# cwkd/BiGCN

Measured on AMD Instinct MI355X. Metric: propagation-trees/sec fwd+bwd, batch=128, 5000-dim feats @ 1/2/4/8 MI355X, higher is better.
Workload: dtype f32

## Files before the change

### bigcn_amd/csrc/bgcn_csc_body.h

```cpp
#pragma once

#include "bgcn_internal.h"
#include "bgcn_sparse.h"

namespace bgcn {

__device__ __forceinline__ int spill_row_of(const int* pre, int nrows, int e) {
  int lo = 0, hi = nrows - 1;
  while (lo < hi) {
    const int mid = (lo + hi + 1) >> 1;
    if (pre[mid] <= e) lo = mid; else hi = mid - 1;
  }
  return lo;
}
template <class Fn>
__device__ __forceinline__ void for_spill(const SparseState& S, const int* pre, const int* off, int nrows,
                                          Fn f) {
  const int total = pre[nrows];
  for (int e0 = int(threadIdx.x); e0 < total; e0 += 4 * int(blockDim.x)) {
    int r[4];
    uint2 v[4];
#pragma unroll
    for (int u = 0; u < 4; ++u) {
      const int e = min(e0 + u * int(blockDim.x), total - 1);
      r[u] = spill_row_of(pre, nrows, e);
      v[u] = S.ovf[off[r[u]] + (e - pre[r[u]])];
    }
#pragma unroll
    for (int u = 0; u < 4; ++u)
      if (e0 + u * int(blockDim.x) < total) f(r[u], v[u]);
  }
}

__device__ inline void csc_hist_body(const SparseState& S, int bid, int32_t* hsm) {
  if (!use_sparse(S)) return;
  for (int64_t c = threadIdx.x; c < S.F; c += kRowBlock) hsm[c] = 0;
  const int64_t i = int64_t(bid) * kRowBlock + threadIdx.x;
  const int64_t ic = min<int64_t>(i, S.N - 1);
  const int nall = i < S.N ? S.nnz[ic] : 0;
  const int n = min(nall, kCap);
  int32_t cl[kCap];
#pragma unroll
  for (int q = 0; q < kCap / 4; ++q) {
    const int4 v = *reinterpret_cast<const int4*>(S.cols + ic * kCap + 4 * q);
    cl[4 * q] = v.x; cl[4 * q + 1] = v.y; cl[4 * q + 2] = v.z; cl[4 * q + 3] = v.w;
  }
  __syncthreads();
#pragma unroll
  for (int s = 0; s < kCap; ++s)
    if (s < n) atomicAdd(&hsm[cl[s]], 1);
  const int nsp = nall > kCap ? nall - kCap : 0;
  if (__syncthreads_or(nsp)) {
    __shared__ int pre[kRowBlock + 1], off[kRowBlock], wsum[kRowBlock / 64];
    const int lane = threadIdx.x & 63, wv = threadIdx.x >> 6;
    int x = nsp;
#pragma unroll
    for (int o = 1; o < 64; o <<= 1) {
      const int y = __shfl_up(x, o, 64);
      if (lane >= o) x += y;
    }
    if (lane == 63) wsum[wv] = x;
    __syncthreads();
    int base = 0, total = 0;
#pragma unroll
    for (int w = 0; w < kRowBlock / 64; ++w) {
      base += w < wv ? wsum[w] : 0;
      total += wsum[w];
    }
    pre[threadIdx.x] = base + x - nsp;
    off[threadIdx.x] = nsp ? S.ovf_off[ic] : 0;
    if (threadIdx.x == 0) pre[kRowBlock] = total;
    __syncthreads();
    for_spill(S, pre, off, kRowBlock, [&](int, uint2 v) { atomicAdd(&hsm[v.x], 1); });
  }
  __syncthreads();
  int32_t* out = S.hist + int64_t(bid) * S.F;
  for (int64_t c = threadIdx.x; c < S.F; c += kRowBlock) out[c] = hsm[c];
}

constexpr int kPrefixCols = 16, kPrefixSegs = 256 / kPrefixCols;
__device__ inline void csc_prefix_body(const SparseState& S, int R, int bid) {
  if (!use_sparse(S)) return;
  __shared__ int32_t part[kPrefixSegs][kPrefixCols];
  const int cl = threadIdx.x % kPrefixCols, q = threadIdx.x / kPrefixCols;
  const int64_t c = min<int64_t>(int64_t(bid) * kPrefixCols + cl, S.F - 1);
  const bool live = int64_t(bid) * kPrefixCols + cl < S.F;
  const int rq = (R + kPrefixSegs - 1) / kPrefixSegs, rb = q * rq, re = min(R, rb + rq);
  int32_t sum = 0;
  for (int r0 = rb; r0 < re; r0 += 8) {
    int32_t v[8];
#pragma unroll
    for (int u = 0; u < 8; ++u) v[u] = S.hist[int64_t(max(min(r0 + u, re - 1), 0)) * S.F + c];
#pragma unroll
    for (int u = 0; u < 8; ++u) sum += r0 + u < re ? v[u] : 0;
  }
  part[q][cl] = sum;
  __syncthreads();
  int32_t run = 0;
  for (int qq = 0; qq < q; ++qq) run += part[qq][cl];
  for (int r0 = rb; r0 < re; r0 += 8) {
    int32_t v[8];
#pragma unroll
    for (int u = 0; u < 8; ++u) v[u] = S.hist[int64_t(max(min(r0 + u, re - 1), 0)) * S.F + c];
#pragma unroll
    for (int u = 0; u < 8; ++u) {
      if (live && r0 + u < re) S.hist[int64_t(r0 + u) * S.F + c] = run;
      run += r0 + u < re ? v[u] : 0;
    }
  }
  if (live && q == kPrefixSegs - 1) S.col_total[c] = run;
}

__device__ inline void csc_colscan_body(const SparseState& S) {
  if (!use_sparse(S)) return;
  __shared__ int32_t wsum[1024];
  const int64_t F = S.F;
  const int nth = int(blockDim.x);
  const int64_t per = (F + nth - 1) / nth;
  const int64_t c0 = threadIdx.x * per;
  constexpr int kMaxPer = kSparseMaxF / 256;
  int32_t v[kMaxPer];
  int32_t local = 0;
#pragma unroll
  for (int k = 0; k < kMaxPer; ++k) {
    const int64_t c = c0 + k;
    v[k] = (k < per && c < F) ? S.col_total[min<int64_t>(c, F - 1)] : 0;
    local += v[k];
  }
  wsum[threadIdx.x] = local;
  __syncthreads();
  for (int o = 1; o < nth; o <<= 1) {
    const int32_t t = threadIdx.x >= o ? wsum[threadIdx.x - o] : 0;
    __syncthreads();
    wsum[threadIdx.x] += t;
    __syncthreads();
  }
  int32_t run = wsum[threadIdx.x] - local;
#pragma unroll
  for (int k = 0; k < kMaxPer; ++k) {
    const int64_t c = c0 + k;
    if (k < per && c < F) {
      S.col_start[c] = run;
      S.col_end[c] = run + v[k];
    }
    run += v[k];
  }
}


__device__ inline void csc_place_body(const SparseState& S, int bid, int32_t* psm) {
  if (!use_sparse(S)) return;
  bid = xcd_contig(bid, int((S.N + kRowBlock - 1) / kRowBlock));
  int32_t* cnt = psm;
  uint32_t* rows = reinterpret_cast<uint32_t*>(psm + S.F);
  const int64_t F = S.F;
  const int32_t* pre = S.hist + int64_t(bid) * F;
  for (int64_t c0 = threadIdx.x; c0 < F; c0 += 4 * 256) {
    int32_t st[4], pr[4];
#pragma unroll
    for (int u = 0; u < 4; ++u) {
      const int64_t c = min<int64_t>(c0 + 256 * u, F - 1);
      st[u] = S.col_start[c];
      pr[u] = pre[c];
    }
#pragma unroll
    for (int u = 0; u < 4; ++u) {
      const int64_t c = c0 + 256 * u;
      if (c < F) {
        cnt[c] = st[u] + pr[u];
        rows[c] = 0u;
      }
    }
  }
  const int64_t r0 = int64_t(bid) * kRowBlock;
  const int s = threadIdx.x % kCap;
  constexpr int kPer = kRowBlock * kCap / 256;
  int32_t col[kPer], nn[kPer];
  float val[kPer];
  uint32_t rootbits = 0u;
#pragma unroll
  for (int k = 0; k < kPer; ++k) {
    const int64_t ic = min<int64_t>(r0 + threadIdx.x / kCap + 8 * k, S.N - 1);
    nn[k] = S.nnz[ic];
    col[k] = S.cols[ic * kCap + s];
    val[k] = S.vals[ic * kCap + s];
    rootbits |= uint32_t(S.root_map[ic] == int32_t(ic)) << k;
  }
  uint32_t smask = 0u;
#pragma unroll
  for (int k = 0; k < kPer; ++k) {
    const int64_t i = r0 + threadIdx.x / kCap + 8 * k;
    col[k] = (i < S.N && s < nn[k]) ? col[k] : -1;
    smask |= (i < S.N && nn[k] > kCap) ? (1u << (k / 4)) : 0u;
  }
  constexpr int kPlaceStage = 1024;
  __shared__ int rpre[kRowBlock + 1], roff[kRowBlock], wsum[kRowBlock / 64];
  __shared__ uint32_t rslot[kRowBlock];
  __shared__ uint2 sbuf[kPlaceStage];
  __shared__ uint32_t smask_s;
  if (threadIdx.x == 0) smask_s = 0u;
  __syncthreads();
  if (smask) atomicOr(&smask_s, smask);
  __syncthreads();
  smask = smask_s;
  bool staged = true;
  if (smask) {
    const int t = threadIdx.x, lane = t & 63, wv = t >> 6;
    const int64_t i = r0 + t;
    const int na = i < S.N ? S.nnz[i] : 0;
    const int nsp = na > kCap ? na - kCap : 0;
    const int o = nsp ? S.ovf_off[i] : 0;
    const uint32_t sl = nsp ? (uint32_t(i * kCap) | kCscSpillFlag | (S.root_map[i] == int32_t(i) ? kCscRootFlag : 0u))
                            : 0u;
    int x = nsp;
#pragma unroll
    for (int d = 1; d < 64; d <<= 1) {
      const int y = __shfl_up(x, d, 64);
      if (lane >= d) x += y;
    }
    if (lane == 63) wsum[wv] = x;
    __syncthreads();
    int base = 0, total = 0;
#pragma unroll
    for (int w = 0; w < kRowBlock / 64; ++w) {
      base += w < wv ? wsum[w] : 0;
      total += wsum[w];
    }
    rpre[t] = base + x - nsp;
    roff[t] = o;
    rslot[t] = sl;
    if (t == 0) rpre[kRowBlock] = total;
    staged = total <= kPlaceStage;
    __syncthreads();
    if (staged) {
      for (int e0 = t; e0 < total; e0 += 4 * kRowBlock) {
        uint2 v[4];
#pragma unroll
        for (int u = 0; u < 4; ++u) {
          const int e = min(e0 + u * kRowBlock, total - 1);
          const int r = spill_row_of(rpre, kRowBlock, e);
          v[u] = S.ovf[roff[r] + (e - rpre[r])];
        }
#pragma unroll
        for (int u = 0; u < 4; ++u)
          if (e0 + u * kRowBlock < total) sbuf[e0 + u * kRowBlock] = v[u];
      }
    }
    __syncthreads();
  }
  auto batch_spill = [&](int bt, auto f) {
    const int lo0 = bt * 32, e1 = rpre[lo0 + 32];
    for (int e = rpre[lo0] + int(threadIdx.x); e < e1; e += int(blockDim.x)) {
      int lo = lo0, hi = lo0 + 31;
      while (lo < hi) {
        const int mid = (lo + hi + 1) >> 1;
        if (rpre[mid] <= e) lo = mid; else hi = mid - 1;
      }
      const uint2 v = staged ? sbuf[e] : S.ovf[roff[lo] + (e - rpre[lo])];
      f(lo - lo0, v, lo);
    }
  };
  constexpr int kBatchRows = 32;
#pragma unroll
  for (int bt = 0; bt < kRowBlock / kBatchRows; ++bt) {
    int rr[4], rank[4];
    const bool spill = (smask >> bt) & 1u;
#pragma unroll
    for (int k = 0; k < 4; ++k) {
      rr[k] = threadIdx.x / kCap + 8 * k;
      const int32_t cc = col[4 * bt + k];
      if (cc >= 0) atomicOr(&rows[cc], 1u << rr[k]);
    }
    if (spill) batch_spill(bt, [&](int r, uint2 v, int) { atomicOr(&rows[v.x], 1u << r); });
    __syncthreads();
#pragma unroll
    for (int k = 0; k < 4; ++k) {
      const int32_t cc = col[4 * bt + k];
      rank[k] = -1;
      if (cc >= 0) {
        const uint32_t m = rows[cc];
        rank[k] = __popc(m & ((1u << rr[k]) - 1u));
        const int64_t i = r0 + bt * kBatchRows + rr[k];
        const uint32_t flag = ((rootbits >> (4 * bt + k)) & 1u) ? kCscRootFlag : 0u;
        S.csc[cnt[cc] + rank[k]] = make_uint2(uint32_t(i * kCap + s) | flag, __float_as_uint(val[4 * bt + k]));
      }
    }
    if (spill)
      batch_spill(bt, [&](int r, uint2 v, int br) {
        S.csc[cnt[v.x] + __popc(rows[v.x] & ((1u << r) - 1u))] = make_uint2(rslot[br], v.y);
      });
    __syncthreads();
    if (!spill) {
#pragma unroll
      for (int k = 0; k < 4; ++k) {
        const int32_t cc = col[4 * bt + k];
        if (rank[k] == 0) {
          cnt[cc] += __popc(rows[cc]);
          rows[cc] = 0u;
        }
      }
    } else {
#pragma unroll
      for (int k = 0; k < 4; ++k)
        if (rank[k] == 0) cnt[col[4 * bt + k]] += __popc(rows[col[4 * bt + k]]);
      batch_spill(bt, [&](int r, uint2 v, int) {
        if ((rows[v.x] & ((1u << r) - 1u)) == 0u) cnt[v.x] += __popc(rows[v.x]);
      });
      __syncthreads();
#pragma unroll
      for (int k = 0; k < 4; ++k)
        if (rank[k] >= 0) rows[col[4 * bt + k]] = 0u;
      batch_spill(bt, [&](int, uint2 v, int) { rows[v.x] = 0u; });
    }
    __syncthreads();
  }
}

}
```

### bigcn_amd/csrc/bgcn_prep.hip

```cpp
#include <cstdlib>
#include <cstring>

#include "bgcn_compact_body.h"
#include "bgcn_csc_body.h"
#include "bgcn_drop_body.h"
#include "bgcn_graph_body.h"
#include "bgcn_internal.h"
#include "bgcn_items_body.h"
#include "bgcn_sparse.h"

namespace bgcn {
namespace {

struct PrepArgs {
  SparseState S;
  GraphBatch gb;
  DropList dl[2];
  const int64_t *batch, *rootindex;
  int32_t *node_root, *tree_ptr, *status;
  const void* X;
  int64_t ldx;
  const int32_t *xr_ptr, *xr_col;
  const float* xr_val;
  uint64_t* span;
  int64_t* eptr;
  uint64_t seed;
  uint4* zero[2];
  int nzero[2];
  int nz, nRP, nR, nbd[2], lists;
  int nsel, ncomp;
  int nce, R;
  int ntile, nprefix;
  int ne, nn, np;
};

__global__ __launch_bounds__(256) void k_prep_a(PrepArgs a) {
  int b = int(blockIdx.x);
  if (b < a.nz) {
    const int64_t w = int64_t(b) * 256 + threadIdx.x;
    const int64_t w0 = a.nzero[0];
    if (w < w0) a.zero[0][w] = make_uint4(0u, 0u, 0u, 0u);
    else if (w - w0 < a.nzero[1]) a.zero[1][w - w0] = make_uint4(0u, 0u, 0u, 0u);
    return;
  }
  b -= a.nz;
  if (b < a.nRP) {
    prologue_batch_body(a.S, a.batch, a.rootindex, a.node_root, a.tree_ptr, b, a.nR);
    return;
  }
  b -= a.nRP;
  const int d = b < a.nbd[0] ? 0 : 1;
  drop_bounds_body(a.dl[d], d, a.batch, a.S.N, a.S.B, a.eptr, a.status, d == 0 ? b : b - a.nbd[0]);
}

template <class TX>
__device__ inline void prep_b_body(const PrepArgs& a) {
  int b = int(blockIdx.x);
  if (b < a.nsel) {
    const int d = b / int(a.S.B);
    drop_select_body(a.dl[d], d, int64_t(b % int(a.S.B)), a.batch, a.S.N, a.S.B, a.seed, a.eptr, 1,
                     nullptr, a.status);
    return;
  }
  b -= a.nsel;
  if (b == 0) {
    items_body(a.S, a.tree_ptr, a.rootindex);
    return;
  }
  if (a.xr_ptr) csr_ell_body(a.S, a.xr_ptr, a.xr_col, a.xr_val, b - 1, a.ncomp);
  else compact_body<false, TX>(a.S, static_cast<const TX*>(a.X), a.ldx, nullptr, b - 1, a.ncomp);
}

#ifndef BGCN_PREP_B_WAVES
#define BGCN_PREP_B_WAVES 2
#endif
template <class TX>
__device__ __forceinline__ void prep_b_stamped(const PrepArgs& a) {
  if (a.span && threadIdx.x == 0 && blockIdx.x < kSpanStarts)
    a.span[blockIdx.x] = uint64_t(wall_clock64());
  prep_b_body<TX>(a);
  if (a.span) {
    __syncthreads();
    if (threadIdx.x == 0)
      atomicMax(reinterpret_cast<unsigned long long*>(a.span) + kSpanStarts + blockIdx.x % kSpanEnds,
                static_cast<unsigned long long>(wall_clock64()));
  }
}

template <class TX>
__global__ __launch_bounds__(256, BGCN_PREP_B_WAVES) void k_prep_b(PrepArgs a) {
  prep_b_stamped<TX>(a);
}

template <class TX>
__global__ __launch_bounds__(256, 3) void k_prep_b_alone(PrepArgs a) {
  prep_b_stamped<TX>(a);
}

__global__ __launch_bounds__(256) void k_prep_select(PrepArgs a) {
  const int b = int(blockIdx.x);
  if (b >= a.nsel) return;
  const int d = b / int(a.S.B);
  drop_select_body(a.dl[d], d, int64_t(b % int(a.S.B)), a.batch, a.S.N, a.S.B, a.seed, a.eptr, 1, nullptr,
                   a.status);
}

__global__ __launch_bounds__(256) void k_prep_f_graph(PrepArgs a) {
  const int per = a.ne + a.nn + a.np;
  const int b = int(blockIdx.x);
  if (b < 2 * per) graph_rank_norm_body(a.gb, a.gb.g[b / per], b % per, a.ne, a.nn);
}

__global__ __launch_bounds__(256) void k_prep_c(PrepArgs a) {
  extern __shared__ __attribute__((aligned(16))) int32_t dsm[];
  int b = int(blockIdx.x);
  if (b < 2 * a.nce) {
    graph_count_body(a.gb, a.gb.g[b / a.nce], b % a.nce);
    return;
  }
  csc_hist_body(a.S, b - 2 * a.nce, dsm);
}

__global__ __launch_bounds__(256) void k_prep_d(PrepArgs a) {
  int b = int(blockIdx.x);
  if (b < 2 * a.ntile) {
    graph_scan_body(a.gb, a.gb.g[b / a.ntile]);
    return;
  }
  csc_prefix_body(a.S, a.R, b - 2 * a.ntile);
}

__global__ __launch_bounds__(256) void k_prep_e(PrepArgs a) {
  int b = int(blockIdx.x);
  const int per = a.ne + a.nn;
  if (b < 2 * per) {
    graph_fill_nodes_body(a.gb, a.gb.g[b / per], b % per, a.ne);
    return;
  }
  csc_colscan_body(a.S);
}

#ifndef BGCN_PREP_F_WAVES
#define BGCN_PREP_F_WAVES 2
#endif
__global__ __launch_bounds__(256, BGCN_PREP_F_WAVES) void k_prep_f(PrepArgs a) {
  extern __shared__ __attribute__((aligned(16))) int32_t dsm[];
  int b = int(blockIdx.x);
  const int per = a.ne + a.nn + a.np;
  if (b < 2 * per) {
    graph_rank_norm_body(a.gb, a.gb.g[b / per], b % per, a.ne, a.nn);
    return;
  }
  csc_place_body(a.S, b - 2 * per, dsm);
}

}

#ifndef BGCN_PREP_LANES_DEFAULT
#define BGCN_PREP_LANES_DEFAULT 2
#endif
void bind_prepared(const Prepared& p, SparseState& S) {
  S.item_tree = p.item_tree; S.tree_item0 = p.tree_item0;
  S.item_beg = p.item_beg; S.item_end = p.item_end; S.item_root = p.item_root;
  S.hist = p.hist; S.col_total = p.col_total; S.col_start = p.col_start; S.col_end = p.col_end;
  S.csc = p.csc;
  S.ovf_off = p.x_ovf_off; S.ovf = p.x_ovf; S.ovf_cap = p.ovf_cap; S.long_rows = p.x_long;
}

static void prepared_state(const Prepared& p, int64_t N, int64_t B, int64_t F, int mode, SparseState& S) {
  S.mode = mode;
  S.N = N; S.F = F; S.B = B;
  S.max_items = int(N / kChunk + B + 1);
  S.flags = p.x_flags; S.nnz = p.x_nnz; S.cols = p.x_cols; S.vals = p.x_vals;
  bind_prepared(p, S);
  S.root_map = p.node_root;
  S.bstatus = p.status;
}

int prep_pipeline(const Prepared& p, const bgcn_batch* bt, int64_t F, int degree_on, int mode,
                  hipStream_t s, bool paced, int nlanes) {
  const int64_t N = bt->num_nodes, B = bt->num_graphs;
  BGCN_CHECK_HIP(hipMemsetAsync(p.status, 0, sizeof(int32_t), s));
  PrepArgs a{};
  SparseState& S = a.S;
  prepared_state(p, N, B, F, mode, S);
  a.batch = bt->batch; a.rootindex = bt->rootindex;
  a.node_root = p.node_root; a.tree_ptr = p.tree_ptr; a.status = p.status;
  a.X = bt->x; a.ldx = bt->ldx;
  if (!bt->x) { a.xr_ptr = bt->x_row_ptr; a.xr_col = bt->x_col; a.xr_val = bt->x_val; }
  const int64_t Etd = bt->td_num_edges, Ebu = bt->bu_num_edges;
  const bool drop = bt->td_droprate > 0.0 || bt->bu_droprate > 0.0;
  const int64_t* td = bt->td_edge_index;
  const int64_t* bu = bt->bu_edge_index;
  a.lists = drop ? 2 : 0;
  if (drop) {
    BGCN_CHECK_ARG(p.dws && p.dws_bytes >= drop_ws_size(B), "drop workspace too small");
    Carve c(p.dws, p.dws_bytes);
    a.eptr = c.take<int64_t>(size_t(2 * (B + 1)));
    a.dl[0] = DropList{td, Etd, p.td_drop, Etd, bt->td_droprate, 0u};
    a.dl[1] = DropList{bu, Ebu, p.bu_drop, Ebu, bt->bu_droprate, 1u};
    a.seed = bt->drop_seed;
    if (td) td = p.td_drop;
    if (bu) bu = p.bu_drop;
  }
  GraphArgs ga[2];
  graph_pair_args(td, Etd, bu, Ebu, &p.td, &p.bu, p.status, p.gws, p.gws_bytes, ga);
  size_t zb[2] = {0, 0};
  BGCN_TRY(graph_batch_setup(ga, 2, N, degree_on, &a.gb, zb, bt->batch));
  for (int k = 0; k < 2; ++k) {
    a.zero[k] = reinterpret_cast<uint4*>(a.gb.g[k].cnt_t);
    a.nzero[k] = int(zb[k] / 16);
    BGCN_CHECK_ARG(zb[k] % 16 == 0 && (reinterpret_cast<uintptr_t>(a.zero[k]) & 15) == 0, "zero range");
  }
  const bool xp = mode != 1;
  const int64_t Emax = std::max(Etd, Ebu);
  a.nz = int((a.nzero[0] + a.nzero[1] + 255) / 256);
  a.nR = int((N + 255) / 256);
  a.nRP = a.nR + int((B + 1 + 255) / 256);
  a.nbd[0] = drop ? int(Etd / 256 + 1) : 0;
  a.nbd[1] = drop ? int(Ebu / 256 + 1) : 0;
  a.nsel = drop ? int(2 * B) : 0;
  {
    static const int ncu = [] {
      int dev = 0, n = 0;
      if (hipGetDevice(&dev) != hipSuccess ||
          hipDeviceGetAttribute(&n, hipDeviceAttributeMultiprocessorCount, dev) != hipSuccess)
        n = 256;
      return n > 0 ? n : 256;
    }();
    const bool bf = bt->x_dtype == BGCN_DTYPE_BF16;
    a.ncomp = xp ? int(grid_for(N, bf ? 8 : 4)) : 0;
    const int paced_cap = bf ? (compact_by_prefix<bf16_t>() ? ncu : 0) : ncu + ncu / 2;
    const int cap = int(knob("BGCN_PREP_BLOCKS", paced ? paced_cap : 0));
    if (cap > 0) a.ncomp = std::min(a.ncomp, cap);
    if (a.xr_ptr && xp) a.ncomp = int(grid_for(N, 8));
  }
  a.nce = graph_edge_blocks(Emax);
  a.R = xp ? int((N + kRowBlock - 1) / kRowBlock) : 0;
  a.ntile = int(graph_scan_tiles(N));
  a.nprefix = xp ? int(grid_for(F, kPrefixCols)) : 0;
  a.ne = graph_edge_blocks(Emax);
  a.nn = graph_node_blocks(N);
  a.np = graph_pos_blocks(Emax, N);
  const dim3 blk(256);
  const bool bf16 = bt->x_dtype == BGCN_DTYPE_BF16;
  void (*const prep_b)(PrepArgs) = paced ? (bf16 ? k_prep_b<bf16_t> : k_prep_b<float>)
                                         : (bf16 ? k_prep_b_alone<bf16_t> : k_prep_b_alone<float>);
  hipLaunchKernelGGL(k_prep_a, dim3(unsigned(a.nz + a.nRP + a.nbd[0] + a.nbd[1])), blk, 0, s, a);
  BGCN_CHECK_LAUNCH();
  const size_t hist_smem = xp ? size_t(F) * sizeof(int32_t) : 0;
  const int default_lanes = int(BGCN_KNOB_ONCE("BGCN_PREP_LANES", BGCN_PREP_LANES_DEFAULT));
  const int lanes = nlanes > 0 ? nlanes : default_lanes;
  if (lanes == 2 && xp) {
    hipStream_t g = s;
    BGCN_TRY(aux_fork(s, kLaneGraph, &g));
    PrepArgs ag = a;
    ag.ncomp = 0; ag.R = 0; ag.nprefix = 0;
    PrepArgs ax = a;
    ax.nsel = 0; ax.nce = 0; ax.ntile = 0; ax.ne = 0; ax.nn = 0; ax.np = 0;
    if (ag.nsel > 0) {
      hipLaunchKernelGGL(k_prep_select, dim3(unsigned(ag.nsel)), blk, 0, g, ag);
      BGCN_CHECK_LAUNCH();
    }
    if (ag.nce > 0) hipLaunchKernelGGL(k_prep_c, dim3(unsigned(2 * ag.nce)), blk, 0, g, ag);
    if (ag.ntile > 0) hipLaunchKernelGGL(k_prep_d, dim3(unsigned(2 * ag.ntile)), blk, 0, g, ag);
    if (ag.ne + ag.nn > 0) hipLaunchKernelGGL(k_prep_e, dim3(unsigned(2 * (ag.ne + ag.nn))), blk, 0, g, ag);
    if (ag.ne + ag.nn + ag.np > 0)
      hipLaunchKernelGGL(k_prep_f_graph, dim3(unsigned(2 * (ag.ne + ag.nn + ag.np))), blk, 0, g, ag);
    BGCN_CHECK_LAUNCH();
    timing_begin(7, s);
    ax.span = span_slot(7);
    hipLaunchKernelGGL(prep_b, dim3(unsigned(1 + ax.ncomp)), blk, 0, s, ax);
    BGCN_CHECK_LAUNCH();
    timing_end(7, s);
    hipLaunchKernelGGL(k_prep_c, dim3(unsigned(ax.R)), blk, hist_smem, s, ax);
    hipLaunchKernelGGL(k_prep_d, dim3(unsigned(ax.nprefix)), blk, 0, s, ax);
    hipLaunchKernelGGL(k_prep_e, dim3(1u), blk, 0, s, ax);
    hipLaunchKernelGGL(k_prep_f, dim3(unsigned(ax.R)), blk, 2 * hist_smem, s, ax);
    BGCN_CHECK_LAUNCH();
    BGCN_TRY(aux_join(s, kLaneGraph));
    return BGCN_OK;
  }
  timing_begin(7, s);
  a.span = span_slot(7);
  hipLaunchKernelGGL(prep_b, dim3(unsigned(a.nsel + 1 + a.ncomp)), blk, 0, s, a);
  BGCN_CHECK_LAUNCH();
  timing_end(7, s);
  if (2 * a.nce + a.R > 0) {
    hipLaunchKernelGGL(k_prep_c, dim3(unsigned(2 * a.nce + a.R)), blk, hist_smem, s, a);
    BGCN_CHECK_LAUNCH();
  }
  hipLaunchKernelGGL(k_prep_d, dim3(unsigned(2 * a.ntile + a.nprefix)), blk, 0, s, a);
  BGCN_CHECK_LAUNCH();
  hipLaunchKernelGGL(k_prep_e, dim3(unsigned(2 * (a.ne + a.nn) + (xp ? 1 : 0))), blk, 0, s, a);
  BGCN_CHECK_LAUNCH();
  hipLaunchKernelGGL(k_prep_f, dim3(unsigned(2 * (a.ne + a.nn + a.np) + a.R)), blk, 2 * hist_smem, s, a);
  BGCN_CHECK_LAUNCH();
  return BGCN_OK;
}

}
```

Baseline: 516,400.

## Replace two-pass CSC column scan with single-pass decoupled look-back scan

Merges the per-column prefix over row-block histograms and the cross-column exclusive scan into a single kernel. It uses a decoupled look-back with atomic ticket ordering, storing flag words in the col_total buffer, which is zeroed by the existing prep_a zero pass. This removes the single-block serial column scan that used to run in k_prep_e and saves one dependent launch in the aux path. The cost is spin-waiting between blocks and extra hist re-reads. A timeout path sets an internal status flag if a predecessor never publishes.

New measurement: 514,300. No clear change (-0.4%).

```diff
diff --git a/bigcn_amd/csrc/bgcn_csc_body.h b/bigcn_amd/csrc/bgcn_csc_body.h
--- a/bigcn_amd/csrc/bgcn_csc_body.h
+++ b/bigcn_amd/csrc/bgcn_csc_body.h
@@ -1,5 +1,6 @@
 #pragma once
 
+#include "bgcn_graph_body.h"
 #include "bgcn_internal.h"
 #include "bgcn_sparse.h"
 
@@ -147,6 +148,98 @@
   }
 }
 
+__host__ __device__ inline int64_t csc_scan_words(int64_t F) { return (F + kPrefixCols - 1) / kPrefixCols + 1; }
+static_assert(kPrefixCols >= 4, "the look-back words fit the [F] int32 array they are carved as");
+__device__ inline void csc_scan_body(const SparseState& S, int R, uint64_t* lb) {
+  if (!use_sparse(S)) return;
+  __shared__ int32_t part[kPrefixSegs][kPrefixCols];
+  __shared__ int ticket;
+  const int nblk = int((S.F + kPrefixCols - 1) / kPrefixCols);
+  if (threadIdx.x == 0) ticket = atomicAdd(reinterpret_cast<int32_t*>(lb + nblk), 1);
+  __syncthreads();
+  const int bid = ticket;
+  const int cl = threadIdx.x % kPrefixCols, q = threadIdx.x / kPrefixCols;
+  const int64_t c = min<int64_t>(int64_t(bid) * kPrefixCols + cl, S.F - 1);
+  const bool live = int64_t(bid) * kPrefixCols + cl < S.F;
+  const int rq = (R + kPrefixSegs - 1) / kPrefixSegs, rb = q * rq, re = min(R, rb + rq);
+  int32_t sum = 0;
+  for (int r0 = rb; r0 < re; r0 += 8) {
+    int32_t v[8];
+#pragma unroll
+    for (int u = 0; u < 8; ++u) v[u] = S.hist[int64_t(max(min(r0 + u, re - 1), 0)) * S.F + c];
+#pragma unroll
+    for (int u = 0; u < 8; ++u) sum += r0 + u < re ? v[u] : 0;
+  }
+  part[q][cl] = live ? sum : 0;
+  __syncthreads();
+  const int lane = threadIdx.x & 63;
+  int32_t tot = 0, cex = 0, agg = 0;
+  if (threadIdx.x < 64) {
+#pragma unroll
+    for (int qq = 0; qq < kPrefixSegs; ++qq) tot += lane < kPrefixCols ? part[qq][lane % kPrefixCols] : 0;
+    int32_t inc = tot;
+#pragma unroll
+    for (int o = 1; o < kPrefixCols; o <<= 1) {
+      const int32_t y = __shfl_up(inc, o, 64);
+      if (lane >= o) inc += y;
+    }
+    cex = inc - tot;
+    agg = __shfl(inc, kPrefixCols - 1, 64);
+    if (lane == 0)
+      __hip_atomic_store(lb + bid, (bid == 0 ? kLbInc : kLbAgg) | uint64_t(uint32_t(agg)), __ATOMIC_RELAXED,
+                         __HIP_MEMORY_SCOPE_AGENT);
+  }
+  int32_t run = 0;
+  for (int qq = 0; qq < q; ++qq) run += part[qq][cl];
+  for (int r0 = rb; r0 < re; r0 += 8) {
+    int32_t v[8];
+#pragma unroll
+    for (int u = 0; u < 8; ++u) v[u] = S.hist[int64_t(max(min(r0 + u, re - 1), 0)) * S.F + c];
+#pragma unroll
+    for (int u = 0; u < 8; ++u) {
+      if (live && r0 + u < re) S.hist[int64_t(r0 + u) * S.F + c] = run;
+      run += r0 + u < re ? v[u] : 0;
+    }
+  }
+  if (threadIdx.x >= 64) return;
+  int32_t before = 0;
+  if (bid > 0) {
+    int j = bid - 1;
+    unsigned spins = 0;
+    for (;;) {
+      const int p = j - lane;
+      const uint64_t w = p >= 0 ? __hip_atomic_load(lb + p, __ATOMIC_RELAXED, __HIP_MEMORY_SCOPE_AGENT)
+                                : kLbInc;
+      const uint64_t fl = w >> 62;
+      const uint64_t ready = __ballot(fl != 0), incl = __ballot(fl == 2);
+      const int stop = incl ? __builtin_ctzll(incl) : 64;
+      const uint64_t need = stop >= 63 ? ~0ull : ((2ull << stop) - 1ull);
+      if ((ready & need) != need) {
+        if (++spins > (1u << 22)) {
+          if (lane == 0 && S.bstatus) atomicOr(S.bstatus, kStatusInternal);
+          break;
+        }
+        __builtin_amdgcn_s_sleep(1);
+        continue;
+      }
+      int32_t v = lane <= stop ? int32_t(w & 0x7fffffffu) : 0;
+#pragma unroll
+      for (int o = 32; o > 0; o >>= 1) v += __shfl_xor(v, o, 64);
+      before += v;
+      if (stop < 64) break;
+      j -= 64;
+    }
+    if (lane == 0)
+      __hip_atomic_store(lb + bid, kLbInc | uint64_t(uint32_t(before + agg)), __ATOMIC_RELAXED,
+                         __HIP_MEMORY_SCOPE_AGENT);
+  }
+  const int64_t cc = int64_t(bid) * kPrefixCols + lane;
+  if (lane < kPrefixCols && cc < S.F) {
+    S.col_start[cc] = before + cex;
+    S.col_end[cc] = before + cex + tot;
+  }
+}
+
 
 __device__ inline void csc_place_body(const SparseState& S, int bid, int32_t* psm) {
   if (!use_sparse(S)) return;
diff --git a/bigcn_amd/csrc/bgcn_prep.hip b/bigcn_amd/csrc/bgcn_prep.hip
--- a/bigcn_amd/csrc/bgcn_prep.hip
+++ b/bigcn_amd/csrc/bgcn_prep.hip
@@ -12,6 +12,7 @@
 namespace bgcn {
 namespace {
 
+constexpr int kPrepZero = 3;
 struct PrepArgs {
   SparseState S;
   GraphBatch gb;
@@ -25,8 +26,8 @@
   uint64_t* span;
   int64_t* eptr;
   uint64_t seed;
-  uint4* zero[2];
-  int nzero[2];
+  uint4* zero[kPrepZero];
+  int nzero[kPrepZero];
   int nz, nRP, nR, nbd[2], lists;
   int nsel, ncomp;
   int nce, R;
@@ -37,10 +38,12 @@
 __global__ __launch_bounds__(256) void k_prep_a(PrepArgs a) {
   int b = int(blockIdx.x);
   if (b < a.nz) {
-    const int64_t w = int64_t(b) * 256 + threadIdx.x;
-    const int64_t w0 = a.nzero[0];
-    if (w < w0) a.zero[0][w] = make_uint4(0u, 0u, 0u, 0u);
-    else if (w - w0 < a.nzero[1]) a.zero[1][w - w0] = make_uint4(0u, 0u, 0u, 0u);
+    int64_t w = int64_t(b) * 256 + threadIdx.x;
+#pragma unroll
+    for (int k = 0; k < kPrepZero; ++k) {
+      if (w >= 0 && w < a.nzero[k]) a.zero[k][w] = make_uint4(0u, 0u, 0u, 0u);
+      w -= a.nzero[k];
+    }
     return;
   }
   b -= a.nz;
@@ -127,17 +130,13 @@
     graph_scan_body(a.gb, a.gb.g[b / a.ntile]);
     return;
   }
-  csc_prefix_body(a.S, a.R, b - 2 * a.ntile);
+  csc_scan_body(a.S, a.R, reinterpret_cast<uint64_t*>(a.S.col_total));
 }
 
 __global__ __launch_bounds__(256) void k_prep_e(PrepArgs a) {
   int b = int(blockIdx.x);
   const int per = a.ne + a.nn;
-  if (b < 2 * per) {
-    graph_fill_nodes_body(a.gb, a.gb.g[b / per], b % per, a.ne);
-    return;
-  }
-  csc_colscan_body(a.S);
+  if (b < 2 * per) graph_fill_nodes_body(a.gb, a.gb.g[b / per], b % per, a.ne);
 }
 
 #ifndef BGCN_PREP_F_WAVES
@@ -207,14 +206,20 @@
   graph_pair_args(td, Etd, bu, Ebu, &p.td, &p.bu, p.status, p.gws, p.gws_bytes, ga);
   size_t zb[2] = {0, 0};
   BGCN_TRY(graph_batch_setup(ga, 2, N, degree_on, &a.gb, zb, bt->batch));
-  for (int k = 0; k < 2; ++k) {
-    a.zero[k] = reinterpret_cast<uint4*>(a.gb.g[k].cnt_t);
-    a.nzero[k] = int(zb[k] / 16);
-    BGCN_CHECK_ARG(zb[k] % 16 == 0 && (reinterpret_cast<uintptr_t>(a.zero[k]) & 15) == 0, "zero range");
-  }
   const bool xp = mode != 1;
+  void* const zp[kPrepZero] = {a.gb.g[0].cnt_t, a.gb.g[1].cnt_t, p.col_total};
+  const size_t zbytes[kPrepZero] = {zb[0], zb[1], xp ? align_up(size_t(csc_scan_words(F)) * 8, 16) : 0};
+  BGCN_CHECK_ARG(zbytes[2] <= size_t(F) * sizeof(int32_t), "look-back words");
+  int64_t zwords = 0;
+  for (int k = 0; k < kPrepZero; ++k) {
+    a.zero[k] = reinterpret_cast<uint4*>(zp[k]);
+    a.nzero[k] = int(zbytes[k] / 16);
+    zwords += a.nzero[k];
+    BGCN_CHECK_ARG(zbytes[k] % 16 == 0 && zbytes[k] / 16 < (size_t(1) << 31) &&
+                       (reinterpret_cast<uintptr_t>(a.zero[k]) & 15) == 0, "zero range");
+  }
   const int64_t Emax = std::max(Etd, Ebu);
-  a.nz = int((a.nzero[0] + a.nzero[1] + 255) / 256);
+  a.nz = int((zwords + 255) / 256);
   a.nR = int((N + 255) / 256);
   a.nRP = a.nR + int((B + 1 + 255) / 256);
   a.nbd[0] = drop ? int(Etd / 256 + 1) : 0;
@@ -275,7 +280,6 @@
     timing_end(7, s);
     hipLaunchKernelGGL(k_prep_c, dim3(unsigned(ax.R)), blk, hist_smem, s, ax);
     hipLaunchKernelGGL(k_prep_d, dim3(unsigned(ax.nprefix)), blk, 0, s, ax);
-    hipLaunchKernelGGL(k_prep_e, dim3(1u), blk, 0, s, ax);
     hipLaunchKernelGGL(k_prep_f, dim3(unsigned(ax.R)), blk, 2 * hist_smem, s, ax);
     BGCN_CHECK_LAUNCH();
     BGCN_TRY(aux_join(s, kLaneGraph));
@@ -292,8 +296,10 @@
   }
   hipLaunchKernelGGL(k_prep_d, dim3(unsigned(2 * a.ntile + a.nprefix)), blk, 0, s, a);
   BGCN_CHECK_LAUNCH();
-  hipLaunchKernelGGL(k_prep_e, dim3(unsigned(2 * (a.ne + a.nn) + (xp ? 1 : 0))), blk, 0, s, a);
-  BGCN_CHECK_LAUNCH();
+  if (a.ne + a.nn > 0) {
+    hipLaunchKernelGGL(k_prep_e, dim3(unsigned(2 * (a.ne + a.nn))), blk, 0, s, a);
+    BGCN_CHECK_LAUNCH();
+  }
   hipLaunchKernelGGL(k_prep_f, dim3(unsigned(2 * (a.ne + a.nn + a.np) + a.R)), blk, 2 * hist_smem, s, a);
   BGCN_CHECK_LAUNCH();
   return BGCN_OK;
```
